# domkirke/acids_transforms

Measured on AMD Instinct MI355X. Metric: spectrogram frames/sec (fwd+invert), n_fft=1024 hop=256, higher is better.
Workload: dtype f32; 1 GPU; configs[1]: batch=1024 clips/GPU x 4 s mono 44.1 kHz, STFT fwd + Magnitude(mel=128, log1p, unipolar) [one fused kernel] + ISTFT invert, fp32; n_fft=1024, hop=256, frames_per_clip=690, clips_per_gpu=1024

## Files before the change

### acids_transforms_amd/csrc/fft512.h

```cpp
#pragma once
#include <hip/hip_runtime.h>
#include <stdint.h>

#include "fastmath.h"
#include "inv1024_pairs.h"

namespace at_hip {

#ifndef AT_WAVE_PRIORITY
#define AT_WAVE_PRIORITY 1
#endif
template <int LEVEL>
__device__ __forceinline__ void wave_priority() {
#if AT_WAVE_PRIORITY
  __builtin_amdgcn_s_setprio(LEVEL);
#endif
}

constexpr int kFftLdsFloat2PerWave = 568;

constexpr int kTwiddleCount = 22 * 64;
constexpr int kTileCtrSlots = 4096;

__device__ __forceinline__ float2 cadd(float2 a, float2 b) { return make_float2(a.x + b.x, a.y + b.y); }
// ... 84 lines not shown
  v[3] = rot_fma<INV>(b6, u7, rr);
  v[7] = rot_fms<INV>(b6, u7, rr);
}

#ifndef AT_LDS_NOMERGE
#define AT_LDS_NOMERGE 1
#endif
template <typename T>
__device__ __forceinline__ T lds_read_single(const T* p) {
#if AT_LDS_NOMERGE
  typedef const volatile __attribute__((address_space(3))) T* lds_ptr;
  return *(lds_ptr)(p);
#else
  return *p;
#endif
}

__device__ __forceinline__ void wave_lds_sync() {
  __builtin_amdgcn_fence(__ATOMIC_RELEASE, "wavefront");
  __builtin_amdgcn_wave_barrier();
  __builtin_amdgcn_fence(__ATOMIC_ACQUIRE, "wavefront");
}

struct Twiddles {
  v2f t1[7];
  v2f t2[7];
  v2f tr[8];
  v2f tr_self;
  __device__ __forceinline__ v2f get1(int k) const { return t1[k]; }
  __device__ __forceinline__ v2f get2(int k) const { return t2[k]; }
  __device__ __forceinline__ v2f getr(int m) const { return tr[m]; }
  __device__ __forceinline__ v2f getr_self() const { return tr_self; }
};

template <bool INV>
struct LdsTwiddles {
  const float2* tab;
  int lane;
  __device__ __forceinline__ v2f get1(int k) const { return lds_read_single(reinterpret_cast<const v2f*>(tab) + k * 64 + lane); }
  __device__ __forceinline__ v2f get2(int k) const { return lds_read_single(reinterpret_cast<const v2f*>(tab) + (7 + k) * 64 + lane); }
  __device__ __forceinline__ v2f getr(int m) const { return lds_read_single(reinterpret_cast<const v2f*>(tab) + (14 + m) * 64 + lane); }
  __device__ __forceinline__ v2f getr_self() const { return lds_read_single(reinterpret_cast<const v2f*>(tab) + (14 + inv1024::kSelfPairedRow) * 64); }
};
struct HybridTwiddles {
  v2f t1[7];
  v2f t2[7];
  const float2* tab;
  int col;
  __device__ __forceinline__ v2f get1(int k) const { return t1[k]; }
  __device__ __forceinline__ v2f get2(int k) const { return t2[k]; }
  __device__ __forceinline__ v2f getr(int m) const { return lds_read_single(reinterpret_cast<const v2f*>(tab) + (14 + m) * 64 + col); }
};

template <bool INV>
__device__ __forceinline__ float2 twiddle_for_lds(const float2* __restrict__ tab, int i) {
  const float2 a = tab[i];
  return (!INV && i >= 14 * 64) ? make_float2(0.5f * a.x, 0.5f * a.y) : a;
}

template <bool INV>
__device__ __forceinline__ void load_twiddles(Twiddles& tw, const float2* __restrict__ tab, int lane) {
#pragma unroll
  for (int k = 0; k < 7; ++k) {
    tw.t1[k] = to_v(tab[k * 64 + lane]);
    tw.t2[k] = to_v(tab[(7 + k) * 64 + lane]);
  }
#pragma unroll
  for (int m = 0; m < 8; ++m) tw.tr[m] = to_v(twiddle_for_lds<INV>(tab, (14 + m) * 64 + lane));
  if (INV) {
    const float2 w = tab[(14 + inv1024::kSelfPairedRow) * 64];
    tw.tr_self = (v2f){__int_as_float(__builtin_amdgcn_readfirstlane(__float_as_int(w.x))),
                       __int_as_float(__builtin_amdgcn_readfirstlane(__float_as_int(w.y)))};
  }
}

#ifndef AT_XCHG1_SWAP
#define AT_XCHG1_SWAP 1
#endif
__device__ __forceinline__ void xchg1_registers(v2f (&v)[8]) {
#pragma unroll
  for (int k = 0; k < 4; ++k)
#pragma unroll
    for (int c = 0; c < 2; ++c) {
      const auto sw = __builtin_amdgcn_permlane32_swap(__float_as_uint(v[k][c]), __float_as_uint(v[k + 4][c]), false, false);
      v[k][c] = __uint_as_float(sw[0]);
      v[k + 4][c] = __uint_as_float(sw[1]);
    }
#pragma unroll
  for (int g = 0; g < 8; g += 4)
#pragma unroll
    for (int k = g; k < g + 2; ++k)
#pragma unroll
      for (int c = 0; c < 2; ++c) {
        const auto sw = __builtin_amdgcn_permlane16_swap(__float_as_uint(v[k][c]), __float_as_uint(v[k + 2][c]), false, false);
        v[k][c] = __uint_as_float(sw[0]);
        v[k + 2][c] = __uint_as_float(sw[1]);
      }
#pragma unroll
  for (int k = 0; k < 8; k += 2)
#pragma unroll
    for (int c = 0; c < 2; ++c) {
      const int a = __float_as_int(v[k][c]), b = __float_as_int(v[k + 1][c]);
      const int a2 = __builtin_amdgcn_update_dpp(a, b, 0x128, 0xf, 0xc, false);
      const int b2 = __builtin_amdgcn_update_dpp(b, a, 0x128, 0xf, 0x3, false);
      v[k][c] = __int_as_float(a2);
      v[k + 1][c] = __int_as_float(b2);
// ... 228 lines not shown
```

### acids_transforms_amd/csrc/fwd1024_forms.h

```cpp
#pragma once

namespace at_hip {
namespace fwd1024 {

constexpr unsigned long long kDefaultBankQuads = 0x001111223ull;
constexpr int kDefaultBankPasses = 9;

struct FwdForm {
  static constexpr bool write_phase = false;
  static constexpr int mel = 0;
  static constexpr int waves = 4;
  static constexpr bool lds_twiddles = false;
  static constexpr int window_passes = 0;
  static constexpr bool polar = false;
  static constexpr int hop_slots = 2;
  static constexpr int hoisted_passes = 0;
  static constexpr int fixed_quads0 = 0, fixed_quads1 = 0;
  static constexpr int fixed_contrast = 1;
  static constexpr bool fixed_power2 = false;
  static constexpr bool aligned_stores = false;
  static constexpr bool nontemporal = false;
  static constexpr int register_tables = 0;
  static constexpr bool persistent = false;
  static constexpr unsigned long long packed_quads = 0;
  static constexpr int packed_passes = 0;
};

template <class Form> constexpr int waves_per_simd() {
  return (Form::lds_twiddles && !Form::window_passes && !Form::register_tables) ? 4 : 3;
}
template <class Form> constexpr int packed_lds_bytes() {
  return Form::packed_quads ? 64 * ((Form::packed_passes + 3) / 4 * 4) * (int)sizeof(int) : 0;
}

struct Plain256 : FwdForm {};
struct Plain128 : FwdForm { static constexpr int hop_slots = 1; };
struct Plain512 : FwdForm { static constexpr int hop_slots = 4; };
struct PhasePlain256 : Plain256 { static constexpr bool write_phase = true; };
struct PhasePlain128 : Plain128 { static constexpr bool write_phase = true; };
struct PhasePlain512 : Plain512 { static constexpr bool write_phase = true; };
struct PlainAligned : FwdForm { static constexpr int waves = 8; static constexpr bool lds_twiddles = true, aligned_stores = true; };
struct PlainAlignedNt : PlainAligned { static constexpr bool nontemporal = true; };
struct PlainAlignedNtPersistent : PlainAlignedNt { static constexpr bool persistent = true; };
struct GenericFeatures256 : FwdForm { static constexpr int mel = 2, waves = 8; static constexpr bool lds_twiddles = true; };
struct GenericFeatures128 : GenericFeatures256 { static constexpr int hop_slots = 1; };
struct GenericFeatures512 : GenericFeatures256 { static constexpr int hop_slots = 4; };
struct GenericSpectrum256 : GenericFeatures256 { static constexpr int mel = 1; };
struct GenericSpectrum128 : GenericFeatures128 { static constexpr int mel = 1; };
struct GenericSpectrum512 : GenericFeatures512 { static constexpr int mel = 1; };
struct PhaseGenericSpectrum256 : GenericSpectrum256 { static constexpr bool write_phase = true; };
struct PhaseGenericSpectrum128 : GenericSpectrum128 { static constexpr bool write_phase = true; };
struct PhaseGenericSpectrum512 : GenericSpectrum512 { static constexpr bool write_phase = true; };
struct ChannelMajor1 : GenericFeatures256 { static constexpr int window_passes = 1; };
struct ChannelMajor2 : GenericFeatures256 { static constexpr int window_passes = 2; };
struct Polar : GenericFeatures256 { static constexpr bool polar = true; };
struct Hoisted1Features : GenericFeatures256 { static constexpr int hoisted_passes = 1; };
struct Hoisted2Features : GenericFeatures256 { static constexpr int hoisted_passes = 2; };
struct Hoisted1Spectrum : Hoisted1Features { static constexpr int mel = 1; };
struct Hoisted2Spectrum : Hoisted2Features { static constexpr int mel = 1; };
struct FixedMel128Spectrum : Hoisted2Spectrum { static constexpr int fixed_quads0 = 8, fixed_quads1 = 2; };
struct FixedMel128SpectrumAligned : FixedMel128Spectrum { static constexpr bool aligned_stores = true; };
struct FixedMel128SpectrumAlignedNt : FixedMel128SpectrumAligned { static constexpr bool nontemporal = true; };
struct FixedMel128SpectrumAlignedNtPersistent : FixedMel128SpectrumAlignedNt { static constexpr bool persistent = true; };
struct FixedMel128Features8Waves : Hoisted2Features { static constexpr int fixed_quads0 = 8, fixed_quads1 = 2; };
struct FixedMel128Features : FixedMel128Features8Waves { static constexpr int waves = 4, register_tables = 3; };
struct LogPowerMel128 : FixedMel128Features { static constexpr int fixed_contrast = 2; static constexpr bool fixed_power2 = true; };
struct MelSpectrogramChannelMajor : FixedMel128Features8Waves {
  static constexpr int waves = 4, window_passes = 2, fixed_contrast = 0;
  static constexpr bool fixed_power2 = true;
};
struct PackedDefaultBankFeatures : GenericFeatures256 {
  static constexpr unsigned long long packed_quads = kDefaultBankQuads;
  static constexpr int packed_passes = kDefaultBankPasses;
};
struct DevFixedMel128SpectrumTables1 : FixedMel128SpectrumAlignedNt { static constexpr int waves = 4, register_tables = 1; };
struct DevFixedMel128SpectrumTables3 : FixedMel128SpectrumAlignedNt { static constexpr int waves = 4, register_tables = 3; };

}

#define AT_FWD1024_FORMS(X)                                                                                          \
  X(Plain128) X(Plain256) X(Plain512) X(PhasePlain128) X(PhasePlain256) X(PhasePlain512)                             \
  X(PlainAligned) X(PlainAlignedNt) X(PlainAlignedNtPersistent)                                                      \
  X(GenericFeatures128) X(GenericFeatures256) X(GenericFeatures512)                                                  \
  X(GenericSpectrum128) X(GenericSpectrum256) X(GenericSpectrum512)                                                  \
  X(PhaseGenericSpectrum128) X(PhaseGenericSpectrum256) X(PhaseGenericSpectrum512)                                   \
  X(ChannelMajor1) X(ChannelMajor2) X(Polar)                                                                         \
  X(Hoisted1Features) X(Hoisted2Features) X(Hoisted1Spectrum) X(Hoisted2Spectrum)                                    \
  X(FixedMel128Spectrum) X(FixedMel128SpectrumAligned) X(FixedMel128SpectrumAlignedNt)                               \
  X(FixedMel128SpectrumAlignedNtPersistent) X(FixedMel128Features8Waves) X(FixedMel128Features)                      \
  X(LogPowerMel128) X(MelSpectrogramChannelMajor) X(PackedDefaultBankFeatures)
#define AT_FWD1024_DEV_FORMS(X) X(DevFixedMel128SpectrumTables1) X(DevFixedMel128SpectrumTables3)

enum Fwd1024Form {
  kFwd1024Rejected = -1,
#define X(F) kFwd##F,
  AT_FWD1024_FORMS(X) AT_FWD1024_DEV_FORMS(X)
#undef X
  kFwd1024Forms,
  kFwd1024ProductForms = kFwdDevFixedMel128SpectrumTables1
};

struct Fwd1024Call {
  int hop;
  bool spectrum, phase, polar, channel_major;
  bool bank;
  int n_passes, n_filters;
  const int* pass_len;
  int contrast;
  bool power2;
  bool out_aligned_512, feat_aligned_16;
  int epilogue;
  int dev_stores = 2;
  bool dev_persistent = false;
  int dev_register_tables = 0;
  bool dev_no_register_tables = false;
};

constexpr int at_hop(int hop, int f128, int f256, int f512) { return hop == 128 ? f128 : hop == 256 ? f256 : f512; }

inline int pick_fwd1024(const Fwd1024Call& c) {
  if (c.hop != 256 && c.hop != 128 && c.hop != 512) return kFwd1024Rejected;
  if (c.hop != 256 && c.bank && (c.polar || c.channel_major)) return kFwd1024Rejected;
  if (c.polar && (!c.bank || c.spectrum)) return kFwd1024Rejected;
  const bool h256 = c.hop == 256;
  const bool aligned = c.dev_stores != 0 && h256 && c.spectrum && !c.phase && !c.polar && c.out_aligned_512;
  const bool nt = c.dev_stores == 2;
  if (!c.bank) {
    if (aligned && nt && c.dev_persistent) return kFwdPlainAlignedNtPersistent;
    if (aligned) return nt ? kFwdPlainAlignedNt : kFwdPlainAligned;
// ... 38 lines not shown
```

### acids_transforms_amd/csrc/stft1024.hip

```cpp
#include <hip/hip_runtime.h>
#include "fastmath.h"
#include <type_traits>
#include <stdint.h>
#include <stdlib.h>
#include <stdio.h>
#include <string.h>
#include <atomic>

#include "band_bank.h"
#include "fft512.h"
#include "fwd1024_forms.h"
#include "run_plan.h"
#include "stft_launch.h"
#include "variants.h"

#ifndef AT_ISTFT_NT
#define AT_ISTFT_NT 1
#endif
#ifndef AT_ISTFT_NTLOAD
#define AT_ISTFT_NTLOAD 1
#endif

namespace at_hip {

constexpr int N = 1024;
constexpr int F = 513;
constexpr int WAVES_PER_BLOCK = 4;

struct FwdParams {
  const float* x;
  const float* window;
  const float2* tw;
  float2* out;
  float* phase;
  long long B, L, clip_stride, T;
  long long total_frames;
  long long frames_per_block;
  int hop;
  int center;
};

__device__ __forceinline__ void load_frame(const FwdParams& p, long long f, int lane, float2 (&v)[8]) {
  const long long b = f / p.T;
  const long long t = f - b * p.T;
  const float* clip = p.x + b * p.clip_stride;
  const long long start = t * (long long)p.hop - (p.center ? N / 2 : 0);
  const bool interior = (start >= 0) && (start + N <= p.L);
  const bool aligned = (((uintptr_t)(clip + start)) & 7) == 0;
  if (interior && aligned) {
    const float2* src = reinterpret_cast<const float2*>(clip + start);
#pragma unroll
    for (int m = 0; m < 8; ++m) v[m] = src[lane + 64 * m];
  } else if (interior) {
    const float* src = clip + start;
#pragma unroll
    for (int m = 0; m < 8; ++m) {
      v[m].x = src[2 * (lane + 64 * m)];
      v[m].y = src[2 * (lane + 64 * m) + 1];
    }
  } else {
#pragma unroll
    for (int m = 0; m < 8; ++m) {
      long long i0 = start + 2 * (lane + 64 * m);
      if (p.center) {
        v[m].x = clip[reflect_index(i0, p.L)];
        v[m].y = clip[reflect_index(i0 + 1, p.L)];
      } else {
        v[m].x = (i0 < p.L) ? clip[i0] : 0.0f;
        v[m].y = (i0 + 1 < p.L) ? clip[i0 + 1] : 0.0f;
      }
    }
  }
}
// ... 32 lines not shown
#pragma unroll
    for (int m = 0; m < 8; ++m) row[lane + 64 * m] = v[m];
    if (lane == 0) row[512] = nyq;
    if (WRITE_PHASE) {
      float* prow = p.phase + f * F;
#pragma unroll
      for (int m = 0; m < 8; ++m) prow[lane + 64 * m] = fast_atan2f(v[m].y, v[m].x);
      if (lane == 0) prow[512] = fast_atan2f(nyq.y, nyq.x);
    }
  }
}

struct FwdRunParams {
  const float* x;
  const float* window;
  const float2* tw;
  float2* out;
  float* phase;
  long long B, L, clip_stride, T;
  long long runs_per_clip, frames_per_run;
  BandBank bank;
  float* feat;
  const float* offset;
  const float* scale;
  float eps;
  int contrast;
  int power2;
  int feat_channel_major;
  long long feat_ld, phase_ld;
  const float* ph_offset;
  const float* ph_scale;
  unsigned* tile_ctr;
  unsigned n_tiles;
};

__device__ __forceinline__ float2 load_pair(const float* clip, long long L, long long i0, bool interior, bool aligned,
                                            int lane_off) {
  if (interior) {
    if (aligned) return reinterpret_cast<const float2*>(clip + i0)[lane_off >> 1];
    return make_float2(clip[i0 + lane_off], clip[i0 + lane_off + 1]);
  }
  return make_float2(clip[reflect_index(i0 + lane_off, L)], clip[reflect_index(i0 + lane_off + 1, L)]);
}


__device__ __forceinline__ float fwd_contrast(float v, int mode, float eps) { return band_contrast_fast(v, mode, eps); }

template <class Form>
__global__ __launch_bounds__(64 * Form::waves, fwd1024::waves_per_simd<Form>()) void stft1024_h256_fwd_kernel(FwdRunParams p) {
  constexpr bool WRITE_PHASE = Form::write_phase, TWLDS = Form::lds_twiddles, POLAR = Form::polar;
  constexpr bool AL = Form::aligned_stores, NT = Form::nontemporal, FP2 = Form::fixed_power2, PW = Form::persistent;
  constexpr int MEL = Form::mel, FWD_WAVES = Form::waves, CMBUF = Form::window_passes, HS = Form::hop_slots;
  constexpr int SP = Form::hoisted_passes, FQ0 = Form::fixed_quads0, FQ1 = Form::fixed_quads1, FC = Form::fixed_contrast;
  constexpr int HYB = Form::register_tables, FNP = Form::packed_passes;
  constexpr fqp_t FQP = Form::packed_quads;
  constexpr int H = 128 * HS;
  constexpr int kNP = FQP ? FNP : 1;
  constexpr int kPkStride = (kNP + 3) / 4 * 4;
  constexpr int kTabTw = TWLDS ? kTwiddleCount : 0;
  constexpr int kFeatCarry = FQP ? 128 : 0;
  constexpr int kWaveLds = kFftLdsFloat2PerWave + kFeatCarry;
  __shared__ float2 lds_all[FWD_WAVES * kWaveLds + kTabTw + 512];
  extern __shared__ float4 band_lds[];
  const int lane = threadIdx.x & 63;
  const int wave = __builtin_amdgcn_readfirstlane(threadIdx.x >> 6);
  float2* lds = lds_all + wave * kWaveLds + kFeatCarry;
  float2* tab = lds_all + FWD_WAVES * kWaveLds;
  float2 raw_first[8];
  auto load_first_frame = [&](const long long run, float2 (&raw)[8]) {
    const long long b = run / p.runs_per_clip;
    if (b >= p.B) return;
    const long long t0 = (run - b * p.runs_per_clip) * p.frames_per_run;
    if (t0 >= p.T) return;
    const float* clip = p.x + b * p.clip_stride;
    const bool clip_aligned = ((((uintptr_t)clip) & 7) == 0);
    const long long s0 = t0 * (128 * HS) - 512;
#pragma unroll
    for (int m = 0; m < 8; ++m) {
      const long long i0 = s0 + 128 * m;
      raw[m] = load_pair(clip, p.L, i0, i0 >= 0 && i0 + 128 <= p.L, clip_aligned, 2 * lane);
    }
  };
  if constexpr (!PW) load_first_frame((long long)blockIdx.x * FWD_WAVES + wave, raw_first);
  if (TWLDS)
    for (int i = threadIdx.x; i < kTwiddleCount; i += 64 * FWD_WAVES) tab[i] = twiddle_for_lds<false>(p.tw, i);
  for (int i = threadIdx.x; i < 512; i += 64 * FWD_WAVES)
    tab[kTabTw + i] = reinterpret_cast<const float2*>(p.window)[i];
  float* wlds = reinterpret_cast<float*>(band_lds);
  int* lane_tab = nullptr;
  if (MEL != 0) {
    int table_floats = 0;
    for (int q = 0; q < p.bank.n_passes; ++q) table_floats += 64 * p.bank.pass_len[q];
    for (int i = threadIdx.x; i < table_floats; i += 64 * FWD_WAVES) wlds[i] = p.bank.weights[i];
    lane_tab = reinterpret_cast<int*>(wlds + table_floats);
    for (int i = threadIdx.x; i < 64 * p.bank.n_passes; i += 64 * FWD_WAVES) {
      lane_tab[i] = p.bank.lane_start[i];
      lane_tab[64 * p.bank.n_passes + i] = p.bank.lane_filter[i];
    }
    if constexpr (FQP != 0) {
      int* pk_tab = lane_tab + 2 * 64 * p.bank.n_passes;
      for (int i = threadIdx.x; i < 64 * kNP; i += 64 * FWD_WAVES) {
        const int q = i >> 6, l = i & 63;
        const int f = p.bank.lane_filter[i];
        pk_tab[l * kPkStride + q] = (p.bank.lane_start[i] * 4) | ((f >= 0 ? f * 4 : 0xfff) << 12);
      }
    }
  }
  __shared__ unsigned s_tile[2];
  if (PW && threadIdx.x == 0) s_tile[0] = atomicAdd(p.tile_ctr, 1u);
#if AT_XCHG1_SWAP
  if (MEL != 0) {
    reinterpret_cast<float*>(lds)[512 + lane] = 0.0f;
    reinterpret_cast<float*>(lds)[576 + lane] = 0.0f;
  }
#endif
  __syncthreads();

  int sp_f[SP > 0 ? SP : 1], sp_start[SP > 0 ? SP : 1], sp_quads[SP > 0 ? SP : 1];
  if constexpr (SP > 0) {
#pragma unroll
    for (int q = 0; q < SP; ++q) {
      sp_f[q] = lane_tab[(SP + q) * 64 + lane];
      sp_start[q] = lane_tab[q * 64 + lane];
      sp_quads[q] = p.bank.pass_len[q] >> 2;
    }
  }
  Twiddles tw_regs;
  if (!TWLDS) load_twiddles<false>(tw_regs, p.tw, lane);
  const LdsTwiddles<false> tw_lds = {tab, lane};
  HybridTwiddles tw_hyb;
  if constexpr (TWLDS && (HYB & 1)) {
#pragma unroll
    for (int k = 0; k < 7; ++k) {
      tw_hyb.t1[k] = to_v(p.tw[k * 64 + lane]);
      tw_hyb.t2[k] = to_v(p.tw[(7 + k) * 64 + lane]);
    }
    tw_hyb.tab = tab;
    tw_hyb.col = lane;
  }
  const float2* win = tab + kTabTw;
  v2f win_regs[8];
  if constexpr ((HYB & 2) != 0) {
#pragma unroll
    for (int m = 0; m < 8; ++m) win_regs[m] = to_v(reinterpret_cast<const float2*>(p.window)[lane + 64 * m]);
  }

  const long long L = p.L;
  const int lane2 = 2 * lane;

  auto do_run = [&](const long long run, const bool preloaded) {
  const long long b = run / p.runs_per_clip;
  if (b >= p.B) return;
  const long long r = run - b * p.runs_per_clip;
  const long long t0 = r * p.frames_per_run;
  long long t1 = t0 + p.frames_per_run;
  if (t1 > p.T) t1 = p.T;
  if (t0 >= t1) return;
  const float* clip = p.x + b * p.clip_stride;
  const bool clip_aligned = ((((uintptr_t)clip) & 7) == 0);

  float2 raw[8];
  if (preloaded) {
#pragma unroll
    for (int m = 0; m < 8; ++m) raw[m] = raw_first[m];
  } else {
    load_first_frame(run, raw);
  }
#pragma unroll
  for (int m = 0; m < 8; ++m) asm volatile("" : "+v"(raw[m].x), "+v"(raw[m].y));
  float2* row = p.out + (b * p.T + t0) * F;
  const long long feat_ld = (POLAR && p.feat_ld) ? p.feat_ld : (long long)p.bank.n_filters;
  const long long phase_ld = (POLAR && p.phase_ld) ? p.phase_ld : F;
  float* prow = (WRITE_PHASE || POLAR) ? p.phase + (b * p.T + t0) * phase_ld : nullptr;
  float* frow = (MEL != 0) ? p.feat + (b * p.T + t0) * feat_ld : nullptr;
  int fc = 0, fhead = 0;
  float* fdst = nullptr;
  if constexpr (FQP != 0) {
    const long long fe0 = (b * p.T + t0) * (long long)F;
    fc = (int)(fe0 & 255);
    fhead = fc;
    fdst = p.feat + (fe0 - fc);
  }
  float ph_off = 0.f, ph_sc = 1.f;
  if (POLAR && p.ph_offset) {
    ph_off = *p.ph_offset;
    ph_sc = *p.ph_scale;
  }
  int rot = 0;
  float2* sp = nullptr;
  v2f carry = {0.f, 0.f};
  bool head = true;
  if constexpr (AL) {
    static_assert(MEL != 2 && !WRITE_PHASE && !POLAR && TWLDS, "aligned stream stores: spectrum out, LDS twiddles");
    const long long e0 = (b * p.T + t0) * F;
    rot = (int)(e0 & 63);
    sp = p.out + (e0 - rot) + lane;
  }
  auto put = [&](float2* dst, v2f val) {
    if (NT) __builtin_nontemporal_store(val, reinterpret_cast<v2f*>(dst));
    else *reinterpret_cast<v2f*>(dst) = val;
  };
  long long t_cur = t0;
  float cm[CMBUF ? CMBUF : 1][8];
  int cm_held[CMBUF ? CMBUF : 1];
#pragma unroll
  for (int q = 0; q < (CMBUF ? CMBUF : 1); ++q) {
    cm_held[q] = 0;
#pragma unroll
    for (int k = 0; k < 8; ++k) cm[q][k] = 0.f;
  }
  float mel_off = 0.f, mel_inv = 1.f;
  if (MEL != 0 && p.offset) {
    mel_off = *p.offset;
    mel_inv = 1.0f / *p.scale;
  }

  float2 nyq_pending = make_float2(0.f, 0.f);
  float2* nyq_dst = nullptr;
  auto flush_nyquist = [&]() {
    if (nyq_dst != nullptr && lane == 0) *nyq_dst = nyq_pending;
    if (WRITE_PHASE && nyq_dst != nullptr && lane == 0)
      p.phase[(nyq_dst - p.out)] = fast_atan2f(nyq_pending.y, nyq_pending.x);
  };
  auto frame_body = [&](const float2 (&fresh)[HS]) {
    wave_priority<3>();
    float2 v[8];
#pragma unroll
    for (int m = 0; m < 8; ++m) {
      const v2f w = (HYB & 2) ? win_regs[m] : lds_read_single(reinterpret_cast<const v2f*>(win) + lane + 64 * m);
      v[m] = make_float2(raw[m].x * w.x, raw[m].y * w.y);
    }
#pragma unroll
    for (int m = 0; m < 8 - HS; ++m) raw[m] = raw[m + HS];
#pragma unroll
    for (int k = 0; k < HS; ++k) raw[8 - HS + k] = fresh[k];
    float2 nyq;
    const int col = AL ? ((lane - rot) & 63) : lane;
    {
      v2f z[8];
#pragma unroll
      for (int m = 0; m < 8; ++m) z[m] = to_v(v[m]);
      if constexpr (AL && (HYB & 1)) {
        fft512<false>(z, tw_hyb, lds, lane, col);
        tw_hyb.col = col;
        rfft_merge_rot(z, tw_hyb, lane, rot, col, nyq);
      } else if constexpr (AL) {
        fft512<false>(z, tw_lds, lds, lane, col);
        const LdsTwiddles<false> tw_col = {tab, col};
        rfft_merge_rot(z, tw_col, lane, rot, col, nyq);
      } else if constexpr (TWLDS && (HYB & 1)) {
        fft512<false>(z, tw_hyb, lds, lane);
        rfft_merge(z, tw_hyb, lane, nyq);
      } else if (TWLDS) {
        fft512<false>(z, tw_lds, lds, lane);
        rfft_merge(z, tw_lds, lane, nyq);
      } else {
        fft512<false>(z, tw_regs, lds, lane);
        rfft_merge(z, tw_regs, lane, nyq);
      }
#pragma unroll
      for (int m = 0; m < 8; ++m) v[m] = to_f2(z[m]);
      if constexpr (AL) {
        wave_priority<1>();
        const bool lo = lane < rot;
        const v2f s0 = lo ? carry : z[0];
        if (head) {
          if (!lo) put(sp, s0);
          head = false;
        } else {
          put(sp, s0);
        }
#pragma unroll
        for (int j = 1; j < 8; ++j) put(sp + 64 * j, lo ? z[j - 1] : z[j]);
        carry = lo ? z[7] : (v2f){nyq.x, 0.f};
        if (rot == 63) {
          put(sp + 512, carry);
          sp += 576;
          rot = 0;
        } else {
          sp += 512;
          ++rot;
        }
      }
    }
    if (MEL != 2 && !AL) {
#pragma unroll
      for (int m = 0; m < 8; ++m) row[lane + 64 * m] = v[m];
    }
    if (WRITE_PHASE) {
#pragma unroll
      for (int m = 0; m < 8; ++m) prow[lane + 64 * m] = fast_atan2f(v[m].y, v[m].x);
      prow += F;
    }
    if (POLAR) {
#pragma unroll
      for (int m = 0; m < 8; ++m) {
        float ph = fast_atan2f(v[m].y, v[m].x);
        if (p.ph_offset) ph = (ph - ph_off) / ph_sc;
// ... 393 lines not shown
  return lds_read_single(reinterpret_cast<const v2f*>(win) + lane + 64 * m);
}

template <typename TW>
__device__ __forceinline__ void synth_frame(float2 (&v)[8], float2 x256, const TW& tw, const float2* win,
                                            float2* lds, int lane) {
  v2f z[8];
#pragma unroll
  for (int m = 0; m < 8; ++m) z[m] = to_v(v[m]);
  irfft_split(z, tw, lane, to_v(x256));
  fft512<true>(z, tw, lds, lane);
#pragma unroll
  for (int m = 0; m < 8; ++m) {
    const v2f w = lds_read_single(reinterpret_cast<const v2f*>(win) + lane + 64 * m);
    v[m] = to_f2(z[m] * w);
  }
}

template <int IN_MODE, int DEPTH, bool TWLDS, int HS = 2>
__global__ __launch_bounds__(64 * WAVES_PER_BLOCK, IN_MODE == IN_GL ? 2 : (TWLDS ? 5 : 4) - DEPTH) void istft1024_ola_kernel(InvParams p) {
  constexpr int R = 8 / HS;
  constexpr int C = 4 / HS;
  constexpr int H = 128 * HS;
  constexpr int kFull = (1 << R) - 1;
  __shared__ float2 lds_all[WAVES_PER_BLOCK * kFftLdsFloat2PerWave + 512 + (TWLDS ? kTwiddleCount : 0)];
  const int lane = threadIdx.x & 63;
  const int wave = __builtin_amdgcn_readfirstlane(threadIdx.x >> 6);
  float2* lds = lds_all + wave * kFftLdsFloat2PerWave;
  float2* win = lds_all + WAVES_PER_BLOCK * kFftLdsFloat2PerWave;
  float2* twtab = win + 512;
  for (int i = threadIdx.x; i < 512; i += 64 * WAVES_PER_BLOCK) win[i] = scaled_window(p.window, i);
  if (TWLDS)
    for (int i = threadIdx.x; i < kTwiddleCount; i += 64 * WAVES_PER_BLOCK) twtab[i] = p.tw[i];
  __syncthreads();

  const long long run = (long long)blockIdx.x * WAVES_PER_BLOCK + wave;
  const long long b = run / p.runs_per_clip;
  if (b >= p.B) return;
  const long long r = run - b * p.runs_per_clip;
  const long long nslots = p.T - 1;
  const long long j0 = r * p.slots_per_run;
  long long j1 = j0 + p.slots_per_run;
  if (j1 > nslots) j1 = nslots;
  if (j0 >= j1) return;

  Twiddles tw_regs;
  if (!TWLDS) load_twiddles<true>(tw_regs, p.tw, lane);
  const LdsTwiddles<true> tw_lds = {twtab, lane};
  auto synth = [&](const float2 (&v)[8], float2 x256, v2f (&z)[8]) {
    if (TWLDS) synth_frame_nowin(v, x256, tw_lds, lds, lane, z);
    else synth_frame_nowin(v, x256, tw_regs, lds, lane, z);
  };

  v2f acc[8];
#pragma unroll
  for (int m = 0; m < 8; ++m) acc[m] = (v2f){0.f, 0.f};

  const long long fbase = b * p.T;
  float* yclip = p.y + b * (H * nslots);
  long long t = (j0 + C - (R - 1) > 0) ? j0 + C - (R - 1) : 0;
  const long long t_last = j1 - 1 + C;
  const long long t_have = (t_last < p.T - 1) ? t_last : p.T - 1;

  RawFrame<IN_MODE> q0 = {}, q1 = {};
  if (t <= t_have) load_raw(p, fbase + t, lane, q0);
  if (t + 1 <= t_have) load_raw(p, fbase + t + 1, lane, q1);

  auto consume = [&](const RawFrame<IN_MODE>& q) {
    float2 v[8];
    float2 x256;
    if constexpr (IN_MODE == IN_GL) raw_to_spectrum(q, v, x256, p.gl_mom);
    else raw_to_spectrum(q, v, x256);
    v2f z[8];
    synth(v, x256, z);
#pragma unroll
    for (int m = 0; m < 8; ++m) acc[m] = __builtin_elementwise_fma(z[m], ola_window(win, lane, m), acc[m]);
  };
  auto put_y = [&](float2* dst, float2 val) {
#if AT_ISTFT_NT
    __builtin_nontemporal_store((v2f){val.x, val.y}, reinterpret_cast<v2f*>(dst));
#else
    *dst = val;
#endif
  };
  static_assert(sizeof(v2f) == sizeof(float2), "");
  auto emit = [&](long long j, const float2* env) {
    float2* dst = reinterpret_cast<float2*>(yclip + j * H);
#pragma unroll
    for (int k = 0; k < HS; ++k) {
      const float2 e = env[lane + 64 * k];
      put_y(dst + lane + 64 * k, make_float2(acc[k].x / e.x, acc[k].y / e.y));
    }
  };
  float2 rcp[HS];
  auto emit_fast = [&](long long j) {
    float2* dst = reinterpret_cast<float2*>(yclip + j * H);
#pragma unroll
    for (int k = 0; k < HS; ++k) put_y(dst + lane + 64 * k, make_float2(acc[k].x * rcp[k].x, acc[k].y * rcp[k].y));
  };
  auto advance = [&]() {
#pragma unroll
    for (int m = 0; m < 8 - HS; ++m) acc[m] = acc[m + HS];
#pragma unroll
    for (int m = 8 - HS; m < 8; ++m) acc[m] = (v2f){0.f, 0.f};
  };
  {
    const float2* env_full = reinterpret_cast<const float2*>(p.env + kFull * H);
#pragma unroll
    for (int k = 0; k < HS; ++k) {
      const float2 e = env_full[lane + 64 * k];
      rcp[k] = make_float2(1.0f / e.x, 1.0f / e.y);
    }
  }
  auto generic_step = [&]() {
    if (t <= t_have) {
      const RawFrame<IN_MODE> cur = q0;
      q0 = q1;
      if (t + 2 <= t_have) load_raw(p, fbase + t + 2, lane, q1);
      consume(cur);
    }
    const long long j = t - C;
    if (j >= j0 && j < j1) {
      int mask = 0;
#pragma unroll
      for (int q = 0; q < R; ++q) {
        const long long tt = t - (R - 1) + q;
        if (tt >= 0 && tt < p.T) mask |= 1 << q;
      }
      if (mask == kFull) emit_fast(j);
      else emit(j, reinterpret_cast<const float2*>(p.env + mask * H));
    }
    advance();
    ++t;
  };

  long long fast_begin = j0 + C > R - 1 ? j0 + C : R - 1;
  long long fast_end = (j1 - 1 + C < t_have - 2) ? j1 - 1 + C : t_have - 2;
  while (t < fast_begin && t <= t_last) generic_step();
  if (t <= fast_end) {
    if (DEPTH == 2) {
      auto fast_step = [&](RawFrame<IN_MODE>& q) {
        const RawFrame<IN_MODE> cur = q;
        load_raw(p, fbase + t + 2, lane, q);
        consume(cur);
        emit_fast(t - C);
        advance();
        ++t;
      };
      while (t + 1 <= fast_end) {
        fast_step(q0);
        fast_step(q1);
      }
    } else {
      q1 = {};
      for (; t <= fast_end; ++t) {
        const RawFrame<IN_MODE> cur = q0;
        load_raw(p, fbase + t + 1, lane, q0);
        consume(cur);
        emit_fast(t - C);
        advance();
      }
      q1 = {};
      if (t + 1 <= t_have) load_raw(p, fbase + t + 1, lane, q1);
    }
  }
  while (t <= t_last) generic_step();
}

template <int IN_MODE, int NW, int OCC>
__global__ __launch_bounds__(64 * NW, OCC) void istft1024_tile_kernel(InvParams p) {
  constexpr int HS = 2, R = 4, H = 256;
  constexpr int kFull = (1 << R) - 1;
  static_assert(IN_MODE != IN_GL, "the Griffin-Lim form keeps the long-run kernel");
  __shared__ float2 lds_all[NW * kFftLdsFloat2PerWave + 512];
  __shared__ float4 park_all[NW * 6 * 64];
  const int lane = threadIdx.x & 63;
  const int wave = __builtin_amdgcn_readfirstlane(threadIdx.x >> 6);
  float2* lds = lds_all + wave * kFftLdsFloat2PerWave;
  float2* win = lds_all + NW * kFftLdsFloat2PerWave;

  const long long tile = blockIdx.x;
  const long long b = tile / p.runs_per_clip;
  const long long k = tile - b * p.runs_per_clip;
  const long long n = p.slots_per_run;
  const long long T = p.T;
  const long long tile0 = k * p.frames_per_block;
  long long tile1 = tile0 + p.frames_per_block;
  if (tile1 > T) tile1 = T;
  auto share = [&](int w, long long& a, long long& e) {
    a = tile0 + w * n;
    if (a > tile1) a = tile1;
    e = (w == NW - 1) ? tile1 : a + n;
    if (e > tile1) e = tile1;
  };
  long long ta, tb;
  share(wave, ta, tb);
  bool self_cool = true;
  if (wave < NW - 1) {
    long long a2, e2;
    share(wave + 1, a2, e2);
    self_cool = e2 - a2 < 3;
  }
  long long t_stop = (self_cool && tb > ta) ? tb + 3 : tb;
  if (t_stop > T) t_stop = T;
  const bool parks = wave > 0 && ta > 0;
  const long long pe0 = ta == 0 ? 2 : ta + 3;
  const long long pe1 = tb + 3;

  const long long fbase = b * T;
  float* yclip = p.y + b * (H * (T - 1));
  long long t = ta;
  RawFrame<IN_MODE> q0 = {}, q1 = {};
  if (t < t_stop) load_raw(p, fbase + t, lane, q0);
  if (t + 1 < t_stop) load_raw(p, fbase + t + 1, lane, q1);

  for (int i = threadIdx.x; i < 512; i += 64 * NW) win[i] = scaled_window(p.window, i);
  Twiddles tw;
  load_twiddles<true>(tw, p.tw, lane);
  __syncthreads();

  v2f acc[8];
#pragma unroll
  for (int m = 0; m < 8; ++m) acc[m] = (v2f){0.f, 0.f};
  auto consume = [&](const RawFrame<IN_MODE>& q, v2f (&z)[8]) {
    float2 v[8];
    float2 x256;
    raw_to_spectrum(q, v, x256);
    synth_frame_nowin(v, x256, tw, lds, lane, z);
#pragma unroll
    for (int m = 0; m < 8; ++m) acc[m] = __builtin_elementwise_fma(z[m], ola_window(win, lane, m), acc[m]);
  };
  auto put_y = [&](float2* dst, float2 val) {
    __builtin_nontemporal_store((v2f){val.x, val.y}, reinterpret_cast<v2f*>(dst));
  };
  float2 rcp[HS];
  {
    const float2* env_full = reinterpret_cast<const float2*>(p.env + kFull * H);
#pragma unroll
    for (int kk = 0; kk < HS; ++kk) {
      const float2 e = env_full[lane + 64 * kk];
      rcp[kk] = make_float2(1.0f / e.x, 1.0f / e.y);
    }
  }
  auto emit_regs = [&](long long hp, v2f a0, v2f a1) {
    float2* dst = reinterpret_cast<float2*>(yclip + (hp - 2) * H);
    if (hp >= 3 && hp < T) {
      put_y(dst + lane, make_float2(a0.x * rcp[0].x, a0.y * rcp[0].y));
      put_y(dst + lane + 64, make_float2(a1.x * rcp[1].x, a1.y * rcp[1].y));
    } else {
      int mask = 0;
#pragma unroll
      for (int q = 0; q < R; ++q) {
        const long long tt = hp - (R - 1) + q;
        if (tt >= 0 && tt < T) mask |= 1 << q;
      }
      const float2* env = reinterpret_cast<const float2*>(p.env + mask * H);
      const float2 e0 = env[lane], e1 = env[lane + 64];
      put_y(dst + lane, make_float2(a0.x / e0.x, a0.y / e0.y));
      put_y(dst + lane + 64, make_float2(a1.x / e1.x, a1.y / e1.y));
    }
  };
  auto advance = [&]() {
#pragma unroll
    for (int m = 0; m < 8 - HS; ++m) acc[m] = acc[m + HS];
#pragma unroll
    for (int m = 8 - HS; m < 8; ++m) acc[m] = (v2f){0.f, 0.f};
  };
  float4* park = park_all + wave * 6 * 64 + lane;
  auto generic_step = [&]() {
    const RawFrame<IN_MODE> cur = q0;
    q0 = q1;
    if (t + 2 < t_stop) load_raw(p, fbase + t + 2, lane, q1);
    v2f v[8];
    consume(cur, v);
    const long long i = t - ta;
    if (parks && i < 3 && t < tb) {
      const int base = i == 0 ? 0 : (i == 1 ? 3 : 5);
#pragma unroll
      for (int s = 0; s < 3; ++s)
        if (s < 3 - i) park[(base + s) * 64] = make_float4(v[2 * s].x, v[2 * s].y, v[2 * s + 1].x, v[2 * s + 1].y);
    }
    if (t >= pe0 && t < pe1) emit_regs(t, acc[0], acc[1]);
    advance();
    ++t;
  };

  long long fast_begin = ta + 3 > pe0 ? ta + 3 : pe0;
  if (fast_begin < 3) fast_begin = 3;
  long long fast_end = tb - 1;
  if (fast_end > t_stop - 3) fast_end = t_stop - 3;
  while (t < fast_begin && t < tb) generic_step();
  if (t <= fast_end) {
    auto fast_step = [&](RawFrame<IN_MODE>& q) {
      const RawFrame<IN_MODE> cur = q;
      load_raw(p, fbase + t + 2, lane, q);
      v2f v[8];
      consume(cur, v);
      float2* dst = reinterpret_cast<float2*>(yclip + (t - 2) * H);
      put_y(dst + lane, make_float2(acc[0].x * rcp[0].x, acc[0].y * rcp[0].y));
      put_y(dst + lane + 64, make_float2(acc[1].x * rcp[1].x, acc[1].y * rcp[1].y));
      advance();
      ++t;
    };
    while (t + 1 <= fast_end) {
      fast_step(q0);
      fast_step(q1);
    }
  }
  while (t < tb) generic_step();
  __syncthreads();
  if (self_cool) {
    while (t < t_stop) generic_step();
    if (t_stop == T && T >= pe0 && T < pe1 && t == T) emit_regs(T, acc[0], acc[1]);
  } else if (tb > ta) {
    const float4* nx = park_all + (wave + 1) * 6 * 64 + lane;
    auto add4 = [&](int hop, int s, const float4 pc) {
      acc[2 * hop] = __builtin_elementwise_fma((v2f){pc.x, pc.y}, ola_window(win, lane, 2 * s), acc[2 * hop]);
      acc[2 * hop + 1] = __builtin_elementwise_fma((v2f){pc.z, pc.w}, ola_window(win, lane, 2 * s + 1), acc[2 * hop + 1]);
    };
    add4(0, 0, nx[0 * 64]);
    add4(1, 1, nx[1 * 64]);
    add4(1, 0, nx[3 * 64]);
    add4(2, 2, nx[2 * 64]);
    add4(2, 1, nx[4 * 64]);
    add4(2, 0, nx[5 * 64]);
#pragma unroll
    for (int s = 0; s < 3; ++s)
      if (tb + s >= pe0) emit_regs(tb + s, acc[2 * s], acc[2 * s + 1]);
  }
}

template <int IN_MODE>
__global__ __launch_bounds__(64 * WAVES_PER_BLOCK) void irfft1024_frames_kernel(InvParams p) {
  __shared__ float2 lds_all[WAVES_PER_BLOCK * kFftLdsFloat2PerWave + 512];
  const int lane = threadIdx.x & 63;
  const int wave = threadIdx.x >> 6;
  float2* lds = lds_all + wave * kFftLdsFloat2PerWave;
  float2* win = lds_all + WAVES_PER_BLOCK * kFftLdsFloat2PerWave;
  for (int i = threadIdx.x; i < 512; i += 64 * WAVES_PER_BLOCK) win[i] = scaled_window(p.window, i);
  __syncthreads();
  Twiddles tw;
  load_twiddles<true>(tw, p.tw, lane);
  const long long f_begin = (long long)blockIdx.x * p.frames_per_block;
  long long f_end = f_begin + p.frames_per_block;
  if (f_end > p.total_frames) f_end = p.total_frames;
  for (long long f = f_begin + wave; f < f_end; f += WAVES_PER_BLOCK) {
    float2 v[8];
    float2 x256;
    load_spectrum<IN_MODE>(p, f, lane, v, x256);
    synth_frame(v, x256, tw, win, lds, lane);
    float2* dst = reinterpret_cast<float2*>(p.y + f * N);
#pragma unroll
    for (int m = 0; m < 8; ++m) dst[lane + 64 * m] = v[m];
  }
}

// ... 223 lines not shown
```

Baseline: 456.7 million frames/s.

## Keep ISTFT window in registers and rotate OLA accumulators as a ring

In the ISTFT kernels, the overlap-add window values are loaded once into registers instead of being read from LDS every frame. The fast loop is unrolled four frames deep, with the accumulator array treated as a ring indexed by a compile-time offset, so the per-frame shift of accumulators goes away. The forward path gains optional forms that keep pass-2 twiddles in registers, but these default off. The cost is higher register pressure, which may lower occupancy.

```diff
diff --git a/acids_transforms_amd/csrc/fft512.h b/acids_transforms_amd/csrc/fft512.h
--- a/acids_transforms_amd/csrc/fft512.h
+++ b/acids_transforms_amd/csrc/fft512.h
@@ -160,6 +160,18 @@
   __device__ __forceinline__ v2f getr(int m) const { return lds_read_single(reinterpret_cast<const v2f*>(tab) + (14 + m) * 64 + col); }
 };
 
+template <int NREG>
+struct Pass2RegTwiddles {
+  v2f t2[NREG > 0 ? NREG : 1];
+  const float2* tab;
+  int lane, col;
+  __device__ __forceinline__ v2f get1(int k) const { return lds_read_single(reinterpret_cast<const v2f*>(tab) + k * 64 + lane); }
+  __device__ __forceinline__ v2f get2(int k) const {
+    return k < NREG ? t2[k] : lds_read_single(reinterpret_cast<const v2f*>(tab) + (7 + k) * 64 + lane);
+  }
+  __device__ __forceinline__ v2f getr(int m) const { return lds_read_single(reinterpret_cast<const v2f*>(tab) + (14 + m) * 64 + col); }
+};
+
 template <bool INV>
 __device__ __forceinline__ float2 twiddle_for_lds(const float2* __restrict__ tab, int i) {
   const float2 a = tab[i];
diff --git a/acids_transforms_amd/csrc/fwd1024_forms.h b/acids_transforms_amd/csrc/fwd1024_forms.h
--- a/acids_transforms_amd/csrc/fwd1024_forms.h
+++ b/acids_transforms_amd/csrc/fwd1024_forms.h
@@ -1,4 +1,11 @@
 #pragma once
+
+#ifndef AT_FWD_PASS2_REGISTERS
+#define AT_FWD_PASS2_REGISTERS 0
+#endif
+#ifndef AT_FWD_PLAIN_TABLES
+#define AT_FWD_PLAIN_TABLES 0
+#endif
 
 namespace at_hip {
 namespace fwd1024 {
@@ -21,13 +28,15 @@
   static constexpr bool aligned_stores = false;
   static constexpr bool nontemporal = false;
   static constexpr int register_tables = 0;
+  static constexpr bool tables_keep_fourth_wave = false;
+  static constexpr int pass2_registers = 0;
   static constexpr bool persistent = false;
   static constexpr unsigned long long packed_quads = 0;
   static constexpr int packed_passes = 0;
 };
 
 template <class Form> constexpr int waves_per_simd() {
-  return (Form::lds_twiddles && !Form::window_passes && !Form::register_tables) ? 4 : 3;
+  return (Form::lds_twiddles && !Form::window_passes && (!Form::register_tables || Form::tables_keep_fourth_wave)) ? 4 : 3;
 }
 template <class Form> constexpr int packed_lds_bytes() {
   return Form::packed_quads ? 64 * ((Form::packed_passes + 3) / 4 * 4) * (int)sizeof(int) : 0;
@@ -39,7 +48,10 @@
 struct PhasePlain256 : Plain256 { static constexpr bool write_phase = true; };
 struct PhasePlain128 : Plain128 { static constexpr bool write_phase = true; };
 struct PhasePlain512 : Plain512 { static constexpr bool write_phase = true; };
-struct PlainAligned : FwdForm { static constexpr int waves = 8; static constexpr bool lds_twiddles = true, aligned_stores = true; };
+struct PlainAligned : FwdForm {
+  static constexpr int waves = 8, register_tables = AT_FWD_PLAIN_TABLES;
+  static constexpr bool lds_twiddles = true, aligned_stores = true, tables_keep_fourth_wave = true;
+};
 struct PlainAlignedNt : PlainAligned { static constexpr bool nontemporal = true; };
 struct PlainAlignedNtPersistent : PlainAlignedNt { static constexpr bool persistent = true; };
 struct GenericFeatures256 : FwdForm { static constexpr int mel = 2, waves = 8; static constexpr bool lds_twiddles = true; };
@@ -60,8 +72,14 @@
 struct Hoisted2Spectrum : Hoisted2Features { static constexpr int mel = 1; };
 struct FixedMel128Spectrum : Hoisted2Spectrum { static constexpr int fixed_quads0 = 8, fixed_quads1 = 2; };
 struct FixedMel128SpectrumAligned : FixedMel128Spectrum { static constexpr bool aligned_stores = true; };
-struct FixedMel128SpectrumAlignedNt : FixedMel128SpectrumAligned { static constexpr bool nontemporal = true; };
-struct FixedMel128SpectrumAlignedNtPersistent : FixedMel128SpectrumAlignedNt { static constexpr bool persistent = true; };
+struct FixedMel128SpectrumAlignedNt : FixedMel128SpectrumAligned {
+  static constexpr bool nontemporal = true;
+  static constexpr int pass2_registers = AT_FWD_PASS2_REGISTERS;
+};
+struct FixedMel128SpectrumAlignedNtPersistent : FixedMel128SpectrumAlignedNt {
+  static constexpr bool persistent = true;
+  static constexpr int pass2_registers = 0;
+};
 struct FixedMel128Features8Waves : Hoisted2Features { static constexpr int fixed_quads0 = 8, fixed_quads1 = 2; };
 struct FixedMel128Features : FixedMel128Features8Waves { static constexpr int waves = 4, register_tables = 3; };
 struct LogPowerMel128 : FixedMel128Features { static constexpr int fixed_contrast = 2; static constexpr bool fixed_power2 = true; };
@@ -73,8 +91,8 @@
   static constexpr unsigned long long packed_quads = kDefaultBankQuads;
   static constexpr int packed_passes = kDefaultBankPasses;
 };
-struct DevFixedMel128SpectrumTables1 : FixedMel128SpectrumAlignedNt { static constexpr int waves = 4, register_tables = 1; };
-struct DevFixedMel128SpectrumTables3 : FixedMel128SpectrumAlignedNt { static constexpr int waves = 4, register_tables = 3; };
+struct DevFixedMel128SpectrumTables1 : FixedMel128SpectrumAlignedNt { static constexpr int waves = 4, register_tables = 1, pass2_registers = 0; };
+struct DevFixedMel128SpectrumTables3 : FixedMel128SpectrumAlignedNt { static constexpr int waves = 4, register_tables = 3, pass2_registers = 0; };
 
 }
 
diff --git a/acids_transforms_amd/csrc/stft1024.hip b/acids_transforms_amd/csrc/stft1024.hip
--- a/acids_transforms_amd/csrc/stft1024.hip
+++ b/acids_transforms_amd/csrc/stft1024.hip
@@ -19,6 +19,12 @@
 #endif
 #ifndef AT_ISTFT_NTLOAD
 #define AT_ISTFT_NTLOAD 1
+#endif
+#ifndef AT_ISTFT_WINDOW_REGS
+#define AT_ISTFT_WINDOW_REGS 1
+#endif
+#ifndef AT_ISTFT_RING4
+#define AT_ISTFT_RING4 1
 #endif
 
 namespace at_hip {
@@ -157,7 +163,8 @@
   constexpr bool AL = Form::aligned_stores, NT = Form::nontemporal, FP2 = Form::fixed_power2, PW = Form::persistent;
   constexpr int MEL = Form::mel, FWD_WAVES = Form::waves, CMBUF = Form::window_passes, HS = Form::hop_slots;
   constexpr int SP = Form::hoisted_passes, FQ0 = Form::fixed_quads0, FQ1 = Form::fixed_quads1, FC = Form::fixed_contrast;
-  constexpr int HYB = Form::register_tables, FNP = Form::packed_passes;
+  constexpr int HYB = Form::register_tables, FNP = Form::packed_passes, P2R = Form::pass2_registers;
+  static_assert(P2R == 0 || (P2R <= 7 && Form::aligned_stores && TWLDS && !(HYB & 1)), "pass-2 rows in registers: the aligned LDS-twiddle forms");
   constexpr fqp_t FQP = Form::packed_quads;
   constexpr int H = 128 * HS;
   constexpr int kNP = FQP ? FNP : 1;
@@ -243,6 +250,14 @@
     tw_hyb.tab = tab;
     tw_hyb.col = lane;
   }
+  Pass2RegTwiddles<P2R> tw_p2;
+  if constexpr (P2R > 0) {
+#pragma unroll
+    for (int k = 0; k < P2R; ++k) tw_p2.t2[k] = to_v(p.tw[(7 + k) * 64 + lane]);
+    tw_p2.tab = tab;
+    tw_p2.lane = lane;
+    tw_p2.col = lane;
+  }
   const float2* win = tab + kTabTw;
   v2f win_regs[8];
   if constexpr ((HYB & 2) != 0) {
@@ -349,6 +364,10 @@
         fft512<false>(z, tw_hyb, lds, lane, col);
         tw_hyb.col = col;
         rfft_merge_rot(z, tw_hyb, lane, rot, col, nyq);
+      } else if constexpr (AL && P2R > 0) {
+        fft512<false>(z, tw_p2, lds, lane, col);
+        tw_p2.col = col;
+        rfft_merge_rot(z, tw_p2, lane, rot, col, nyq);
       } else if constexpr (AL) {
         fft512<false>(z, tw_lds, lds, lane, col);
         const LdsTwiddles<false> tw_col = {tab, col};
@@ -848,6 +867,14 @@
     else synth_frame_nowin(v, x256, tw_regs, lds, lane, z);
   };
 
+  constexpr bool WREG = AT_ISTFT_WINDOW_REGS && IN_MODE != IN_GL && HS == 2 && DEPTH == 2 && !TWLDS;
+  constexpr bool RING4 = AT_ISTFT_RING4 && IN_MODE != IN_GL && HS == 2 && DEPTH == 2 && !TWLDS;
+  v2f win_regs[8];
+  if constexpr (WREG) {
+#pragma unroll
+    for (int m = 0; m < 8; ++m) win_regs[m] = ola_window(win, lane, m);
+  }
+
   v2f acc[8];
 #pragma unroll
   for (int m = 0; m < 8; ++m) acc[m] = (v2f){0.f, 0.f};
@@ -862,7 +889,8 @@
   if (t <= t_have) load_raw(p, fbase + t, lane, q0);
   if (t + 1 <= t_have) load_raw(p, fbase + t + 1, lane, q1);
 
-  auto consume = [&](const RawFrame<IN_MODE>& q) {
+  auto consume = [&](const RawFrame<IN_MODE>& q, auto ring) {
+    constexpr int O = decltype(ring)::value;
     float2 v[8];
     float2 x256;
     if constexpr (IN_MODE == IN_GL) raw_to_spectrum(q, v, x256, p.gl_mom);
@@ -870,8 +898,12 @@
     v2f z[8];
     synth(v, x256, z);
 #pragma unroll
-    for (int m = 0; m < 8; ++m) acc[m] = __builtin_elementwise_fma(z[m], ola_window(win, lane, m), acc[m]);
-  };
+    for (int m = 0; m < 8; ++m) {
+      const v2f w = WREG ? win_regs[m] : ola_window(win, lane, m);
+      acc[(m + O) & 7] = __builtin_elementwise_fma(z[m], w, acc[(m + O) & 7]);
+    }
+  };
+  constexpr std::integral_constant<int, 0> ring0 = {};
   auto put_y = [&](float2* dst, float2 val) {
 #if AT_ISTFT_NT
     __builtin_nontemporal_store((v2f){val.x, val.y}, reinterpret_cast<v2f*>(dst));
@@ -913,7 +945,7 @@
       const RawFrame<IN_MODE> cur = q0;
       q0 = q1;
       if (t + 2 <= t_have) load_raw(p, fbase + t + 2, lane, q1);
-      consume(cur);
+      consume(cur, ring0);
     }
     const long long j = t - C;
     if (j >= j0 && j < j1) {
@@ -938,11 +970,32 @@
       auto fast_step = [&](RawFrame<IN_MODE>& q) {
         const RawFrame<IN_MODE> cur = q;
         load_raw(p, fbase + t + 2, lane, q);
-        consume(cur);
+        consume(cur, ring0);
         emit_fast(t - C);
         advance();
         ++t;
       };
+      if constexpr (RING4) {
+        auto ring_step = [&](RawFrame<IN_MODE>& q, auto ring) {
+          constexpr int O = decltype(ring)::value;
+          const RawFrame<IN_MODE> cur = q;
+          load_raw(p, fbase + t + 2, lane, q);
+          consume(cur, ring);
+          float2* dst = reinterpret_cast<float2*>(yclip + (t - C) * H);
+#pragma unroll
+          for (int k = 0; k < HS; ++k) {
+            put_y(dst + lane + 64 * k, make_float2(acc[(k + O) & 7].x * rcp[k].x, acc[(k + O) & 7].y * rcp[k].y));
+            acc[(k + O) & 7] = (v2f){0.f, 0.f};
+          }
+          ++t;
+        };
+        while (t + 3 <= fast_end) {
+          ring_step(q0, std::integral_constant<int, 0>());
+          ring_step(q1, std::integral_constant<int, 2>());
+          ring_step(q0, std::integral_constant<int, 4>());
+          ring_step(q1, std::integral_constant<int, 6>());
+        }
+      }
       while (t + 1 <= fast_end) {
         fast_step(q0);
         fast_step(q1);
@@ -952,7 +1005,7 @@
       for (; t <= fast_end; ++t) {
         const RawFrame<IN_MODE> cur = q0;
         load_raw(p, fbase + t + 1, lane, q0);
-        consume(cur);
+        consume(cur, ring0);
         emit_fast(t - C);
         advance();
       }
@@ -1018,14 +1071,25 @@
   v2f acc[8];
 #pragma unroll
   for (int m = 0; m < 8; ++m) acc[m] = (v2f){0.f, 0.f};
-  auto consume = [&](const RawFrame<IN_MODE>& q, v2f (&z)[8]) {
+  constexpr bool WREG = AT_ISTFT_WINDOW_REGS && OCC == 2, RING4 = AT_ISTFT_RING4 && OCC == 2;
+  v2f win_regs[8];
+  if constexpr (WREG) {
+#pragma unroll
+    for (int m = 0; m < 8; ++m) win_regs[m] = ola_window(win, lane, m);
+  }
+  auto consume = [&](const RawFrame<IN_MODE>& q, v2f (&z)[8], auto ring) {
+    constexpr int O = decltype(ring)::value;
     float2 v[8];
     float2 x256;
     raw_to_spectrum(q, v, x256);
     synth_frame_nowin(v, x256, tw, lds, lane, z);
 #pragma unroll
-    for (int m = 0; m < 8; ++m) acc[m] = __builtin_elementwise_fma(z[m], ola_window(win, lane, m), acc[m]);
-  };
+    for (int m = 0; m < 8; ++m) {
+      const v2f w = WREG ? win_regs[m] : ola_window(win, lane, m);
+      acc[(m + O) & 7] = __builtin_elementwise_fma(z[m], w, acc[(m + O) & 7]);
+    }
+  };
+  constexpr std::integral_constant<int, 0> ring0 = {};
   auto put_y = [&](float2* dst, float2 val) {
     __builtin_nontemporal_store((v2f){val.x, val.y}, reinterpret_cast<v2f*>(dst));
   };
@@ -1068,7 +1132,7 @@
     q0 = q1;
     if (t + 2 < t_stop) load_raw(p, fbase + t + 2, lane, q1);
     v2f v[8];
-    consume(cur, v);
+    consume(cur, v, ring0);
     const long long i = t - ta;
     if (parks && i < 3 && t < tb) {
       const int base = i == 0 ? 0 : (i == 1 ? 3 : 5);
@@ -1091,13 +1155,34 @@
       const RawFrame<IN_MODE> cur = q;
       load_raw(p, fbase + t + 2, lane, q);
       v2f v[8];
-      consume(cur, v);
+      consume(cur, v, ring0);
       float2* dst = reinterpret_cast<float2*>(yclip + (t - 2) * H);
       put_y(dst + lane, make_float2(acc[0].x * rcp[0].x, acc[0].y * rcp[0].y));
       put_y(dst + lane + 64, make_float2(acc[1].x * rcp[1].x, acc[1].y * rcp[1].y));
       advance();
       ++t;
     };
+    if constexpr (RING4) {
+      auto ring_step = [&](RawFrame<IN_MODE>& q, auto ring) {
+        constexpr int O = decltype(ring)::value;
+        const RawFrame<IN_MODE> cur = q;
+        load_raw(p, fbase + t + 2, lane, q);
+        v2f v[8];
+        consume(cur, v, ring);
+        float2* dst = reinterpret_cast<float2*>(yclip + (t - 2) * H);
+        put_y(dst + lane, make_float2(acc[O].x * rcp[0].x, acc[O].y * rcp[0].y));
+        put_y(dst + lane + 64, make_float2(acc[O + 1].x * rcp[1].x, acc[O + 1].y * rcp[1].y));
+        acc[O] = (v2f){0.f, 0.f};
+        acc[O + 1] = (v2f){0.f, 0.f};
+        ++t;
+      };
+      while (t + 3 <= fast_end) {
+        ring_step(q0, std::integral_constant<int, 0>());
+        ring_step(q1, std::integral_constant<int, 2>());
+        ring_step(q0, std::integral_constant<int, 4>());
+        ring_step(q1, std::integral_constant<int, 6>());
+      }
+    }
     while (t + 1 <= fast_end) {
       fast_step(q0);
       fast_step(q1);
```

Result: no change. 461.1 million frames/s, median of 2 (+1.0%).
